# BraveenSri/siddhi

Measured on AMD Instinct MI355X. Metric: events/sec (whole node) for partitioned pattern query at 1/2/4/8 GPUs; % HBM peak, higher is better.
Workload: dtype f32

## Files before the change

### siddhi_amd/csrc/gwalk.h

```cpp
#pragma once
#include <hip/hip_runtime.h>

#include <algorithm>
#include <cstdlib>
#include <cstring>
#include <type_traits>

#include "keypart.h"
#include "sg_engine.h"
#include "sg_prim.h"
#include "walk.h"

struct GwArgs {
  int64_t n, nc;
  int64_t within;
  int64_t t0;
  uint32_t K, ns1;
  int32_t stack_mode;
  int32_t cap;
  int32_t chunk;
  int32_t carry_out;
  int32_t pzero;
  const uint32_t* o1;
  const PtU4* grec;
  const uint8_t* glk;
  const uint32_t* kbase;
  uint64_t* trig;
  uint32_t epoch;
  uint64_t* area;
  int64_t* cv_ts;
  int32_t* cv_key;
  int64_t* cv_val;
  int64_t* cv_pay;
  uint32_t* cv_n;
  uint32_t cv_cap;
  uint32_t* flags;
  uint32_t* ovf_keys;
  uint32_t* ovf_n;
  uint32_t ovf_cap;
  uint32_t* match_n;
};
static const uint32_t GW_ORDER = 1, GW_OVERFLOW = 2, GW_INTERNAL = 4, GW_CARRY_FULL = 8;

static const uint32_t GW_MATCH_MAX = (1u << 24) - 1;
__device__ __forceinline__ uint64_t gw_trig_word(uint64_t unit, uint32_t m, uint32_t epoch) {
  return unit | ((uint64_t)m << 32) | ((uint64_t)epoch << 56);
}
__device__ __forceinline__ uint32_t gw_trig_matches(uint64_t w, uint32_t epoch) {
  return (uint32_t)(w >> 56) == epoch ? (uint32_t)(w >> 32) & GW_MATCH_MAX : 0u;
}

static __global__ void __launch_bounds__(256) k_gw_count(const uint32_t* __restrict__ o1, uint32_t ns1, uint32_t K,
                                                         const uint8_t* __restrict__ glk, uint32_t* __restrict__ kcnt) {
  __shared__ uint32_t c[4][256];
  const uint32_t g = blockIdx.x, t = threadIdx.x, w = t >> 6;
#pragma unroll
  for (int q = 0; q < 4; ++q) c[q][t] = 0;
  __syncthreads();
  const uint32_t lo = o1[(size_t)g * ns1], hi = o1[(size_t)(g + 1) * ns1];
  for (uint32_t p = lo + t; p < hi; p += 256) atomicAdd(&c[w][glk[p]], 1u);
  __syncthreads();
  const uint32_t k = (g << 8) + t;
  if (k < K) kcnt[k] = c[0][t] + c[1][t] + c[2][t] + c[3][t];
}

template <int PT>
struct GwLds {
  PtU4 stage[256 * PT];
  uint32_t cw[4][256];
  uint32_t ls[256], tot[256];
  uint32_t wsum[4];
};

template <class T>
struct GwLdsRing {
  T* v;
  int32_t* t;
  int32_t* p;
  uint32_t cmask, lane;
  __device__ __forceinline__ uint32_t ix(uint32_t s) const { return (s & cmask) * 256 + lane; }
  __device__ __forceinline__ bool full(uint32_t head, uint32_t top) const { return top - head == cmask + 1; }
};
template <class T>
struct GwHbmRing {
  T* v;
  int32_t* t;
  int32_t* p;
  __device__ __forceinline__ uint32_t ix(uint32_t s) const { return s; }
  __device__ __forceinline__ bool full(uint32_t, uint32_t) const { return false; }
};

template <class T, int OP, bool STACK, class RING>
struct GwLane {
  RING R;
  uint32_t head = 0, top = 0;
  int32_t hts = 0, prev = INT32_MIN;
  T tv = T();
  bool bad = false;
  bool big = false;
  uint64_t cur = 0;
  uint32_t k = 0;
  uint32_t nm = 0;
  uint32_t wi = 0;
  __device__ __forceinline__ bool step(const GwArgs& a, const PtU4& q) {
    const int32_t dts = (int32_t)q.x;
    const uint32_t rowf = q.y;
    T x;
    const uint32_t xb = q.z;
    __builtin_memcpy(&x, &xb, sizeof(T));
    const int32_t pay = (int32_t)q.w;
    const uint32_t f = rowf >> 30;
    bad |= dts < prev;
    prev = dts;
    if (!f) return true;
    const bool live = !is_nan_val<T>(x);
    if (head != top && (uint32_t)(dts - hts) > wi) {
// ... 42 lines not shown
              R.p[wx] = R.p[si];
            }
            ++wr;
          }
        }
        top = wr;
        if (head != top) {
          hts = R.t[R.ix(head)];
          tv = R.v[R.ix(top - 1)];
        }
      }
      if (emit && m) {
        const uint64_t b = r - (uint32_t)a.nc;
        a.area[hdr] = (uint64_t)(uint32_t)dts | ((uint64_t)k << 32);
        a.area[hdr + 1] = (uint64_t)(uint32_t)val_bits<T>(x) | ((uint64_t)(uint32_t)pay << 32);
        big |= m > GW_MATCH_MAX;
        a.trig[b] = gw_trig_word(hdr, m & GW_MATCH_MAX, a.epoch);
        cur = hdr + 2 + m;
        nm += m;
      }
    }
    if ((f & F_CAND) && live) {
      if (R.full(head, top)) return false;
      const uint32_t s = R.ix(top);
      R.v[s] = x;
      R.t[s] = dts;
      R.p[s] = pay;
      if (top == head) hts = dts;
      tv = x;
      ++top;
    }
    return true;
  }
  __device__ __forceinline__ void carry(const GwArgs& a, uint32_t o) const {
    for (uint32_t e = 0; e < top - head; ++e) {
      const uint32_t s = R.ix(head + e);
      a.cv_ts[o + e] = a.t0 + (int64_t)R.t[s];
      a.cv_key[o + e] = (int32_t)k;
      a.cv_val[o + e] = val_bits<T>(R.v[s]);
      a.cv_pay[o + e] = a.pzero ? (int64_t)(uint32_t)R.p[s] : (int64_t)R.p[s];
    }
  }
};

template <class T, int OP, int PT, bool STACK>
__global__ void __launch_bounds__(256, 1) k_gwalk(GwArgs a) {
  extern __shared__ __attribute__((aligned(16))) char lds_raw[];
  GwLds<PT>& L = *(GwLds<PT>*)lds_raw;
  const uint32_t cap = (uint32_t)a.cap;
  const uint32_t t = threadIdx.x, w = t >> 6, lane = t & 63;
  const uint32_t g = xcd_block(blockIdx.x, gridDim.x);
  const uint32_t k = (g << 8) + t;
  const bool active = k < a.K;
  const uint32_t lo = a.o1[(size_t)g * a.ns1], hi = a.o1[(size_t)(g + 1) * a.ns1];
  GwLane<T, OP, STACK, GwLdsRing<T>> W;
  W.R.v = (T*)(lds_raw + sizeof(GwLds<PT>));
  W.R.t = (int32_t*)(W.R.v + (size_t)cap * 256);
  W.R.p = W.R.t + (size_t)cap * 256;
  W.R.cmask = cap - 1;
  W.R.lane = t;
  W.k = k;
  W.wi = a.within > 0xffffffffll ? 0xffffffffu : (uint32_t)a.within;
  W.cur = active ? 3ull * a.kbase[k] : 0ull;
  bool ovf = false;
  const uint32_t ROWS = 256 * PT;
  PtU4 rc[PT], rn[PT];
  uint32_t tg[PT], tn[PT];
  auto load = [&](uint32_t base, PtU4* r, uint32_t* d) {
    const uint32_t rows = min(ROWS, hi - base);
#pragma unroll
    for (int s = 0; s < PT; ++s) {
      const uint32_t i = w * (PT * 64) + s * 64 + lane;
      const uint32_t p = base + (i < rows ? i : rows - 1);
      r[s] = __builtin_nontemporal_load(a.grec + p);
      d[s] = a.glk[p];
    }
  };
  if (lo < hi) load(lo, rc, tg);
  for (uint32_t base = lo; base < hi; base += ROWS) {
    {
      const uint32_t rows = min(ROWS, hi - base);
#pragma unroll
      for (int s = 0; s < PT; ++s)
        if (w * (PT * 64) + s * 64 + lane >= rows) tg[s] = 0xffffffffu;
    }
#pragma unroll
    for (int q = 0; q < 4; ++q) L.cw[q][t] = 0;
    __syncthreads();
#pragma unroll
    for (int s = 0; s < PT; ++s)
      if (tg[s] != 0xffffffffu) atomicAdd(&L.cw[w][tg[s]], 1u);
    __syncthreads();
    {
      const uint32_t c0 = L.cw[0][t], c1 = L.cw[1][t], c2 = L.cw[2][t], c3 = L.cw[3][t];
      const uint32_t tt = c0 + c1 + c2 + c3;
      const uint32_t ex = block_excl_scan256(tt, L.wsum);
      L.ls[t] = ex;
      L.tot[t] = tt;
      L.cw[0][t] = ex;
      L.cw[1][t] = ex + c0;
      L.cw[2][t] = ex + c0 + c1;
      L.cw[3][t] = ex + c0 + c1 + c2;
    }
    __syncthreads();
#pragma unroll
    for (int s = 0; s < PT; ++s) {
      const bool valid = tg[s] != 0xffffffffu;
// ... 9 lines not shown
    if (base + ROWS < hi) load(base + ROWS, rn, tn);
    __syncthreads();
    const uint32_t i0 = L.ls[t], i1 = i0 + L.tot[t];
    for (uint32_t i = i0; i < i1 && active && !ovf; ++i)
      if (!W.step(a, L.stage[i])) ovf = true;
    __syncthreads();
#pragma unroll
    for (int s = 0; s < PT; ++s) { rc[s] = rn[s]; tg[s] = tn[s]; }
  }
  uint32_t fl = W.bad ? GW_ORDER : 0u;
  if (active && W.cur > 3ull * a.kbase[k + 1]) fl |= GW_INTERNAL;
  if (ovf) {
    const uint32_t o = atomicAdd(a.ovf_n, 1u);
    if (o < a.ovf_cap) a.ovf_keys[o] = k;
    else fl |= GW_OVERFLOW;
  }
  if (fl) atomicOr(a.flags, fl);
  {
    uint32_t c = (active && !ovf) ? W.nm : 0u;
#pragma unroll
    for (int o = 32; o > 0; o >>= 1) c += (uint32_t)__shfl_xor((int)c, o);
    if (lane == 0 && c) atomicAdd(a.match_n, c);
  }
  if (!a.carry_out) return;
  const uint32_t m = (active && !ovf) ? W.top - W.head : 0u;
  uint32_t incl = m;
#pragma unroll
  for (int o = 1; o < 64; o <<= 1) {
    const uint32_t y = (uint32_t)__shfl_up((int)incl, o);
    if ((int)lane >= o) incl += y;
  }
  const uint32_t tot = (uint32_t)__shfl((int)incl, 63);
  if (!tot) return;
  uint32_t cb = 0;
  if (lane == 63) cb = atomicAdd(a.cv_n, tot);
  cb = (uint32_t)__shfl((int)cb, 63);
  if ((uint64_t)cb + tot > (uint64_t)a.cv_cap) {
    if (lane == 63) atomicOr(a.flags, GW_CARRY_FULL);
    return;
  }
  if (m) W.carry(a, cb + incl - m);
}

static const uint32_t GW_REDO_LDS = 2048;
template <class T, int OP, bool STACK>
__global__ void __launch_bounds__(256) k_gw_redo(GwArgs a, uint32_t* __restrict__ rows, T* __restrict__ hv,
                                                 int32_t* __restrict__ ht, int32_t* __restrict__ hp) {
  __shared__ uint32_t wc[4], base_s;
  __shared__ PtU4 red_stage[GW_REDO_LDS];
  __shared__ T red_v[GW_REDO_LDS];
  __shared__ int32_t red_t[GW_REDO_LDS], red_p[GW_REDO_LDS];
  const uint32_t k = a.ovf_keys[blockIdx.x];
  const uint32_t g = k >> 8, d = k & 255u, t = threadIdx.x, w = t >> 6, lane = t & 63;
  const uint32_t lo = a.o1[(size_t)g * a.ns1], hi = a.o1[(size_t)(g + 1) * a.ns1];
  const uint32_t kb = a.kbase[k], ke = a.kbase[k + 1];
  if (t == 0) base_s = 0;
  __syncthreads();
  for (uint32_t p0 = lo; p0 < hi; p0 += 256) {
    const uint32_t p = p0 + t;
    const bool mine = p < hi && a.glk[p] == d;
    const uint64_t bm = __ballot(mine);
    const uint32_t below = __builtin_amdgcn_mbcnt_hi((uint32_t)(bm >> 32), __builtin_amdgcn_mbcnt_lo((uint32_t)bm, 0u));
    if (lane == 0) wc[w] = (uint32_t)__popcll(bm);
    __syncthreads();
    uint32_t before = base_s;
    for (uint32_t q = 0; q < w; ++q) before += wc[q];
    if (mine && kb + before + below < ke) rows[kb + before + below] = p;
    __syncthreads();
    if (t == 0) base_s += wc[0] + wc[1] + wc[2] + wc[3];
    __syncthreads();
  }
  const uint32_t nk = ke - kb;
  const bool in_lds = nk <= GW_REDO_LDS;
  if (in_lds)
    for (uint32_t i = t; i < nk; i += 256) red_stage[i] = a.grec[rows[kb + i]];
  __syncthreads();
  if (t != 0) return;
  if (kb + base_s != ke) { atomicOr(a.flags, GW_INTERNAL); return; }
  GwLane<T, OP, STACK, GwHbmRing<T>> W;
  if (in_lds) {
    W.R.v = red_v;
    W.R.t = red_t;
    W.R.p = red_p;
  } else {
    W.R.v = hv + kb;
    W.R.t = ht + kb;
    W.R.p = hp + kb;
  }
  W.k = k;
  W.wi = a.within > 0xffffffffll ? 0xffffffffu : (uint32_t)a.within;
  W.cur = 3ull * kb;
  if (in_lds) for (uint32_t i = 0; i < nk; ++i) W.step(a, red_stage[i]);
  else for (uint32_t i = kb; i < ke; ++i) W.step(a, a.grec[rows[i]]);
  uint32_t fl = W.bad ? GW_ORDER : 0u;
  if (W.cur > 3ull * ke) fl |= GW_INTERNAL;
  if (W.big) fl |= GW_OVERFLOW;
  if (fl) atomicOr(a.flags, fl);
  if (W.nm) atomicAdd(a.match_n, W.nm);
  if (!a.carry_out) return;
  const uint32_t m = W.top - W.head;
  if (!m) return;
  const uint32_t o = atomicAdd(a.cv_n, m);
  if ((uint64_t)o + m > (uint64_t)a.cv_cap) { atomicOr(a.flags, GW_CARRY_FULL); return; }
  W.carry(a, o);
}

struct GwSel {
// ... 158 lines not shown
  const size_t cap = h->ws.bufs[name].bytes;
  if (p != tw.p || cap != tw.cap) {
    tw.p = p;
    tw.cap = cap;
    tw.hw = 0;
  }
  if (wrap && tw.hw) HIPCHK(hipMemsetAsync(p, 0, sizeof(uint64_t) * tw.hw, st));
  if (words > tw.hw) {
    HIPCHK(hipMemsetAsync(p + tw.hw, 0, sizeof(uint64_t) * (words - tw.hw), st));
    tw.hw = words;
  }
  return p;
}

static void gw_project(SgHandle* h, const BatchView& bv, int64_t n, const GwArgs& ga, const GwSel& sel, uint32_t total) {
  const sg_nfa_desc& d = h->desc;
  hipStream_t st = h->stream;
  char* out = h->out.reserve(total, d.n_select, st);
  const int64_t ntile = (n + GW_TILE - 1) / GW_TILE;
  uint32_t* tcount = (uint32_t*)h->ws.get("gw_tcount", sizeof(uint32_t) * ((size_t)ntile + 1), st);
  uint32_t* tbase = (uint32_t*)h->ws.get("gw_tbase", sizeof(uint32_t) * ((size_t)ntile + 1), st);
  h->kbeg("gw_tiles");
  HIPCHK(hipMemsetAsync(tcount + ntile, 0, sizeof(uint32_t), st));
  hipLaunchKernelGGL(k_gtile_count, dim3((unsigned)((ntile + 7) / 8)), dim3(256), 0, st, n, (const uint64_t*)ga.trig, ga.epoch,
                     tcount, ntile);
  HIPCHK(hipGetLastError());
  sg_exclusive_scan(h->ws, st, "gw_tscan_tmp", tcount, tbase, (uint32_t)0, (size_t)ntile + 1, rocprim::plus<uint32_t>());
  h->kend();
  uint32_t tsum = 0;
  HIPCHK(hipMemcpyAsync(&tsum, tbase + ntile, sizeof(uint32_t), hipMemcpyDeviceToHost, st));
  h->kbeg("gw_project");
  const size_t plds = (size_t)GW_PROJ_S * sel.stride;
  if (plds > 65536)
    HIPCHK(hipFuncSetAttribute((const void*)k_gscan_project, hipFuncAttributeMaxDynamicSharedMemorySize, (int)plds));
  hipLaunchKernelGGL(k_gscan_project, dim3((unsigned)ntile), dim3(256), plds, st, n, ga.t0, bv.base_index, bv.index,
                     (const uint64_t*)ga.trig, ga.epoch, (const uint64_t*)ga.area, sel, (int64_t)h->out.n, out,
                     (const uint32_t*)tbase);
  HIPCHK(hipGetLastError());
  h->kend();
  HIPCHK(hipStreamSynchronize(st));
  if (tsum != total) throw SgError(SG_EINVAL, "internal: group walker match count mismatch");
  h->out.n += total;
}

template <class T>
static int run_group_walk(SgHandle* h, const BatchView& bv, int64_t n, int64_t nc, uint32_t kb, const PartPlan& pp,
                          const uint32_t* o1, const WRec<T, true>* grec, const uint8_t* glk, uint32_t* pk_flags,
                          const GwPlan& gp, const PushPlan& plan, const Virt& v, const SgCols& cc, int op, int stack_mode,
                          int val_col_a, EveryNextState* es) {
  const sg_nfa_desc& d = h->desc;
  hipStream_t st = h->stream;
  const int64_t nt = nc + n;
  const uint32_t ng = (kb + 255) >> 8;
  uint32_t* kcnt = (uint32_t*)h->ws.get("gw_kcnt", sizeof(uint32_t) * ((size_t)kb + 1), st);
  uint32_t* kbase = (uint32_t*)h->ws.get("gw_kbase", sizeof(uint32_t) * ((size_t)kb + 1), st);
  h->kbeg("gw_count");
  HIPCHK(hipMemsetAsync(kcnt, 0, sizeof(uint32_t) * ((size_t)kb + 1), st));
  hipLaunchKernelGGL(k_gw_count, dim3(ng), dim3(256), 0, st, o1, pp.ns1, kb, glk, kcnt);
  HIPCHK(hipGetLastError());
  sg_exclusive_scan(h->ws, st, "gw_kscan_tmp", kcnt, kbase, (uint32_t)0, (size_t)kb + 1, rocprim::plus<uint32_t>());
  h->kend();
  uint32_t pkf = 0;
  int64_t t0 = 0;
  HIPCHK(hipMemcpyAsync(&pkf, pk_flags, sizeof(uint32_t), hipMemcpyDeviceToHost, st));
  HIPCHK(hipMemcpyAsync(&t0, nc ? v.c_ts : v.ts, sizeof(int64_t), hipMemcpyDeviceToHost, st));
  HIPCHK(hipStreamSynchronize(st));
  const PackRange pr = pack_range(pkf);
  if (pr == PACK_TS_RANGE) return 2;
  if (pr == PACK_PAY_RANGE) return 0;
  h->mark(2);

  GwArgs ga;
  memset(&ga, 0, sizeof(ga));
  ga.n = n;
  ga.nc = nc;
  ga.within = d.within;
  ga.t0 = t0;
  ga.K = kb;
  ga.ns1 = pp.ns1;
  ga.stack_mode = stack_mode;
  ga.cap = gp.cap;
  ga.chunk = 4096;
  ga.carry_out = h->opt.no_carry ? 0 : 1;
  ga.pzero = v.pfloat;
  ga.o1 = o1;
  ga.grec = (const PtU4*)grec;
  ga.glk = glk;
  ga.kbase = kbase;
  const char* ee = getenv("SG_DEBUG_GW_EPOCHS");
  const uint32_t epochs = ee ? (uint32_t)std::min(std::max(atoi(ee), 1), 255) : 255u;
  const bool wrap = h->gw_epoch >= epochs;
  h->gw_epoch = wrap ? 1u : h->gw_epoch + 1;
  ga.epoch = h->gw_epoch;
  ga.trig = gw_tagged_words(h, h->gw_trig, "gw_trig", (size_t)std::max<int64_t>(n, 1), wrap, st);
  ga.area = (uint64_t*)h->ws.get("gw_area", sizeof(uint64_t) * 3 * (size_t)std::max<int64_t>(nt, 1), st);
  uint32_t* gflags = (uint32_t*)h->ws.get("gw_flags", sizeof(uint32_t) * 4, st);
  ga.flags = gflags;
  ga.cv_n = gflags + 1;
  ga.ovf_n = gflags + 2;
  ga.ovf_cap = std::min<uint32_t>(kb, 1u << 16);
  ga.ovf_keys = (uint32_t*)h->ws.get("gw_ovf_keys", sizeof(uint32_t) * ga.ovf_cap, st);
  ga.match_n = gflags + 3;
  ga.cv_cap = (uint32_t)std::max<int64_t>(1, std::min<int64_t>(nt, (int64_t)kb * gp.cap + (1 << 22)));
  ga.cv_ts = (int64_t*)h->ws.get("cv_ts", sizeof(int64_t) * (size_t)ga.cv_cap, st);
  ga.cv_val = (int64_t*)h->ws.get("cv_val", sizeof(int64_t) * (size_t)ga.cv_cap, st);
  ga.cv_pay = (int64_t*)h->ws.get("cv_pay", sizeof(int64_t) * (size_t)ga.cv_cap, st);
  ga.cv_key = (int32_t*)h->ws.get("cv_key", sizeof(int32_t) * (size_t)ga.cv_cap, st);
  HIPCHK(hipMemsetAsync(gflags, 0, sizeof(uint32_t) * 4, st));
  h->kbeg("group_walk");
  dispatch_op(op, [&](auto opc) { launch_gwalk<T, decltype(opc)::value>(ga, ng, st); });
  h->kend();
  uint32_t hf[4] = {0, 0, 0, 0}, total = 0;
  HIPCHK(hipMemcpyAsync(hf, gflags, sizeof(hf), hipMemcpyDeviceToHost, st));
  HIPCHK(hipStreamSynchronize(st));
  if (hf[0] & GW_INTERNAL) throw SgError(SG_EINVAL, "internal: group walker guard tripped");
  if (hf[0]) return 0;
  if (hf[2]) {
    h->kbeg("gw_redo");
    uint32_t* rrows = (uint32_t*)h->ws.get("gw_redo_rows", sizeof(uint32_t) * (size_t)nt, st);
    char* rl = (char*)h->ws.get("gw_redo_list", (sizeof(T) + 8) * (size_t)nt, st);
    T* hv = (T*)rl;
    int32_t* ht = (int32_t*)(rl + sizeof(T) * (size_t)nt);
    int32_t* hp = ht + nt;
    dispatch_op(op, [&](auto opc) { launch_gw_redo<T, decltype(opc)::value>(ga, hf[2], rrows, hv, ht, hp, st); });
    h->kend();
    HIPCHK(hipMemcpyAsync(hf, gflags, sizeof(hf), hipMemcpyDeviceToHost, st));
    HIPCHK(hipStreamSynchronize(st));
    if (hf[0] & GW_INTERNAL) throw SgError(SG_EINVAL, "internal: group walker redo guard tripped");
    if (hf[0]) return 0;
  }
  h->last_spilled = hf[2];
  total = hf[3];
// ... 28 lines not shown
```

### siddhi_amd/csrc/keypart.h

```cpp
#pragma once
#include <hip/hip_runtime.h>

#include <algorithm>
#include <cstdlib>
#include <cstring>
#include <type_traits>

#include "sg_engine.h"
#include "sg_prim.h"
#include "walk_rec.h"

#ifndef SG_PT1
#define SG_PT1 4
#endif
#ifndef SG_PT2
#define SG_PT2 16
#endif
static const int PT1 = SG_PT1, PT1_ROWS = 256 * SG_PT1;
static const int PT2 = SG_PT2, PT2_ROWS = 256 * SG_PT2;
static const int PT_D = 256;

struct PartPlan {
  uint32_t K, lb, ng, two;
  uint32_t nb1, nb2;
  uint32_t seg1, ns1;
  uint32_t ts2, nj;
};

template <class R, int PT, class TG = uint16_t>
struct PartLds {
  R stage[256 * PT];
  TG tag[256 * PT];
  uint32_t cw[4][PT_D];
  uint32_t ls[PT_D];
  uint32_t tot[PT_D];
  uint32_t run[PT_D];
  uint32_t wsum[4];
};

__device__ __forceinline__ uint32_t block_excl_scan256(uint32_t x, uint32_t* wsum) {
  const int lane = threadIdx.x & 63, w = threadIdx.x >> 6;
  uint32_t inc = x;
#pragma unroll
  for (int o = 1; o < 64; o <<= 1) {
    const uint32_t y = (uint32_t)__shfl_up((int)inc, o);
    if (lane >= o) inc += y;
  }
  if (lane == 63) wsum[w] = inc;
  __syncthreads();
  uint32_t add = 0;
  for (int i = 0; i < w; ++i) add += wsum[i];
  return add + inc - x;
}

__device__ __forceinline__ void peer_rank(bool valid, uint32_t d, uint32_t nb, uint32_t& rank, uint32_t& cnt) {
  uint64_t m = __ballot(valid);
  for (uint32_t b = 0; b < nb; ++b) {
    const bool bit = (d >> b) & 1u;
    const uint64_t bb = __ballot(bit);
    m &= bit ? bb : ~bb;
  }
  rank = __builtin_amdgcn_mbcnt_hi((uint32_t)(m >> 32), __builtin_amdgcn_mbcnt_lo((uint32_t)m, 0u));
  cnt = (uint32_t)__popcll(m);
}

template <class R, int PT, class TG>
__device__ __forceinline__ uint32_t part_cursors(PartLds<R, PT, TG>& L) {
  const uint32_t t = threadIdx.x;
  const uint32_t c0 = L.cw[0][t], c1 = L.cw[1][t], c2 = L.cw[2][t], c3 = L.cw[3][t];
  const uint32_t tot = c0 + c1 + c2 + c3;
  const uint32_t ex = block_excl_scan256(tot, L.wsum);
  L.ls[t] = ex;
  L.tot[t] = tot;
  L.cw[0][t] = ex;
  L.cw[1][t] = ex + c0;
  L.cw[2][t] = ex + c0 + c1;
  L.cw[3][t] = ex + c0 + c1 + c2;
  __syncthreads();
  return L.ls[PT_D - 1] + L.tot[PT_D - 1];
// ... 69 lines not shown
            if (R::has_pay && pk.v.pcol && pk.v.pw == 8) {
              const int64_t pv = v_payload(pk.v, r);
              if (pv != (int64_t)(int32_t)pv) bad |= PK_PAY_RANGE;
            }
          }
        }
      }
    }
  };
  uint32_t tg[P], tn[P];
  R rc[P], rn[P];
  if (rb < re) load(rb, tg, rc);
  for (int64_t base = rb; base < re; base += PROWS) {
#pragma unroll
    for (int q = 0; q < 4; ++q) L.cw[q][t] = 0;
    __syncthreads();
#pragma unroll
    for (int s = 0; s < P; ++s)
      if (tg[s] != 0xffffffffu) atomicAdd(&L.cw[w][tg[s] >> pp.lb], 1u);
    __syncthreads();
    const uint32_t staged = part_cursors(L);
#pragma unroll
    for (int s = 0; s < P; ++s) {
      const bool valid = tg[s] != 0xffffffffu;
      const uint32_t d = valid ? tg[s] >> pp.lb : 0u;
      uint32_t rank, cnt;
      peer_rank(valid, d, pp.nb1, rank, cnt);
      if (valid) {
        const uint32_t slot = L.cw[w][d] + rank;
        if (rank == 0) L.cw[w][d] = slot + cnt;
        L.stage[slot] = rc[s];
        L.tag[slot] = (TG)tg[s];
      }
    }
    if (base + PROWS < re) load(base + PROWS, tn, rn);
    __syncthreads();
    for (uint32_t q = t; q < staged; q += 256) {
      const uint32_t k = L.tag[q], d = k >> pp.lb;
      const uint32_t dst = L.run[d] + q - L.ls[d];
      if ((int64_t)dst >= nt) { bad |= PK_INTERNAL; continue; }
      orec[dst] = L.stage[q];
      if (olk) olk[dst] = (LK)(k & lmask);
    }
    __syncthreads();
    L.run[t] += L.tot[t];
#pragma unroll
    for (int s = 0; s < P; ++s) { tg[s] = tn[s]; rc[s] = rn[s]; }
  }
  if (bad) atomicOr(flags, bad);
}

__device__ __forceinline__ void part2_range(const PartPlan& pp, const uint32_t* o1, uint32_t g, uint32_t jj,
                                            uint32_t& lo, uint32_t& hi) {
  lo = o1[(size_t)g * pp.ns1 + jj * pp.ts2];
  hi = o1[(size_t)g * pp.ns1 + min(pp.ns1, (jj + 1) * pp.ts2)];
}

static __global__ void __launch_bounds__(256) k_part2_hist(PartPlan pp, const uint32_t* __restrict__ o1,
                                                           const uint8_t* __restrict__ glk, uint32_t* __restrict__ h2) {
  __shared__ uint32_t cnt[4][PT_D];
  const uint32_t g = blockIdx.x / pp.nj, jj = blockIdx.x % pp.nj, t = threadIdx.x, w = t >> 6;
#pragma unroll
  for (int q = 0; q < 4; ++q) cnt[q][t] = 0;
  __syncthreads();
  uint32_t lo, hi;
  part2_range(pp, o1, g, jj, lo, hi);
  for (uint32_t pb = lo; pb < hi; pb += 256 * 8) {
    uint32_t d[8];
#pragma unroll
    for (int s = 0; s < 8; ++s) {
      const uint32_t p = pb + s * 256 + t;
      d[s] = p < hi ? (uint32_t)glk[p] : 0xffffffffu;
    }
#pragma unroll
    for (int s = 0; s < 8; ++s)
      if (d[s] != 0xffffffffu) atomicAdd(&cnt[w][d[s]], 1u);
  }
  __syncthreads();
  if (t < (1u << pp.lb)) h2[(size_t)((g << pp.lb) + t) * pp.nj + jj] = cnt[0][t] + cnt[1][t] + cnt[2][t] + cnt[3][t];
}

template <class R>
__global__ void __launch_bounds__(256) k_part2(PartPlan pp, const uint32_t* __restrict__ o1, const uint32_t* __restrict__ o2,
                                               const R* __restrict__ grec, const uint8_t* __restrict__ glk,
                                               R* __restrict__ srec, uint32_t cap, uint32_t* __restrict__ flags) {
  extern __shared__ __attribute__((aligned(16))) char lds_raw[];
  PartLds<R, PT2>& L = *(PartLds<R, PT2>*)lds_raw;
  const uint32_t g = blockIdx.x / pp.nj, jj = blockIdx.x % pp.nj;
  const uint32_t t = threadIdx.x, w = t >> 6, lane = t & 63;
  if (t < (1u << pp.lb)) L.run[t] = o2[(size_t)((g << pp.lb) + t) * pp.nj + jj];
  uint32_t lo, hi;
  part2_range(pp, o1, g, jj, lo, hi);
  auto load = [&](uint32_t base, uint32_t* tg, R* rc) {
    const uint32_t rows = (hi - base < (uint32_t)PT2_ROWS) ? hi - base : (uint32_t)PT2_ROWS;
#pragma unroll
    for (int s = 0; s < PT2; ++s) {
      const uint32_t i = w * (PT2 * 64) + s * 64 + lane;
      const uint32_t p = base + (i < rows ? i : rows - 1);
      const uint32_t lk = glk[p];
      rc[s] = grec[p];
      tg[s] = i < rows ? lk : 0xffffffffu;
    }
  };
  uint32_t tg[PT2], tn[PT2];
  R rc[PT2], rn[PT2];
  if (lo < hi) load(lo, tg, rc);
  for (uint32_t base = lo; base < hi; base += PT2_ROWS) {
#pragma unroll
// ... 15 lines not shown
        if (rank == 0) L.cw[w][d] = slot + cnt;
        L.stage[slot] = rc[s];
        L.tag[slot] = (uint16_t)d;
      }
    }
    if (hi - base > (uint32_t)PT2_ROWS) load(base + PT2_ROWS, tn, rn);
    __syncthreads();
    for (uint32_t q = t; q < staged; q += 256) {
      const uint32_t d = L.tag[q];
      const uint32_t dst = L.run[d] + q - L.ls[d];
      if (dst >= cap) { atomicOr(flags, PK_INTERNAL); continue; }
      srec[dst] = L.stage[q];
    }
    __syncthreads();
    L.run[t] += L.tot[t];
#pragma unroll
    for (int s = 0; s < PT2; ++s) { tg[s] = tn[s]; rc[s] = rn[s]; }
  }
}

typedef uint32_t PtU4 __attribute__((ext_vector_type(4)));
struct PtB24 { uint64_t a, b, c; };
template <class R>
using PtRaw = typename std::conditional<sizeof(R) == 16, PtU4, PtB24>::type;

static __global__ void k_part_segs(uint32_t K, const uint32_t* __restrict__ o, uint32_t stride,
                                   uint32_t* __restrict__ seg_b, uint32_t* __restrict__ seg_e) {
  const uint32_t k = blockIdx.x * blockDim.x + threadIdx.x;
  if (k >= K) return;
  seg_b[k] = o[(size_t)k * stride];
  seg_e[k] = o[(size_t)(k + 1) * stride];
}

static PartPlan part_plan(uint32_t K, int64_t nt) {
  PartPlan p;
  memset(&p, 0, sizeof(p));
  p.K = K;
  uint32_t bits = 0;
  while ((1ull << bits) < (uint64_t)K) ++bits;
  auto nbits = [](uint32_t nd) { uint32_t b = 0; while ((1u << b) < nd) ++b; return b; };
  if (K <= (uint32_t)PT_D) {
    p.two = 0; p.lb = 0; p.ng = K;
  } else {
    const uint32_t hb = (bits + 1) / 2;
    p.two = 1; p.lb = bits - hb; p.ng = (K + (1u << p.lb) - 1) >> p.lb;
  }
  p.nb1 = nbits(p.ng);
  p.nb2 = p.lb;
  const int64_t sub = std::max<int64_t>(1, std::min<int64_t>(32, nt / ((int64_t)PT1_ROWS * 2048)));
  p.seg1 = (uint32_t)(PT1_ROWS * sub);
  p.ns1 = (uint32_t)std::max<int64_t>(1, (nt + p.seg1 - 1) / p.seg1);
  p.ts2 = (uint32_t)std::max<int64_t>(1, std::min<int64_t>(p.ns1, (int64_t)8192 * p.ng / p.seg1));
  p.nj = (p.ns1 + p.ts2 - 1) / p.ts2;
  return p;
}


static __global__ void __launch_bounds__(256) k_hist_wide(KeyOf kf, uint32_t K, uint32_t lb, uint32_t ng, uint32_t seg1,
                                                          uint32_t ns1, int64_t nt, uint32_t* __restrict__ h,
                                                          uint32_t lbs, uint32_t nsg, uint32_t* __restrict__ ha,
                                                          uint32_t* __restrict__ flags) {
  __shared__ uint32_t cnt[4096];
  const uint32_t j = blockIdx.x, t = threadIdx.x;
  for (uint32_t g = t; g < ng; g += 256) cnt[g] = 0;
  __syncthreads();
  const int64_t r0 = (int64_t)j * seg1, r1 = min(nt, r0 + seg1);
  uint32_t bad = 0;
  for (int64_t rb = r0; rb < r1; rb += 256 * 8) {
    uint32_t k[8];
#pragma unroll
    for (int s = 0; s < 8; ++s) {
      const int64_t r = rb + s * 256 + t;
      k[s] = r < r1 ? kf((uint32_t)r) : 0xffffffffu;
    }
#pragma unroll
    for (int s = 0; s < 8; ++s) {
      if (k[s] < K) atomicAdd(&cnt[k[s] >> lb], 1u);
      else if (k[s] != 0xffffffffu) bad |= PK_KEY_RANGE;
    }
  }
  __syncthreads();
  for (uint32_t g = t; g < ng; g += 256) h[(size_t)g * ns1 + j] = cnt[g];
  for (uint32_t sg = t; sg < nsg; sg += 256) {
    uint32_t c = 0;
    for (uint32_t g = sg << lbs; g < ((sg + 1) << lbs) && g < ng; ++g) c += cnt[g];
    ha[(size_t)sg * ns1 + j] = c;
  }
  if (bad) atomicOr(flags, bad);
}

struct Part1bArgs {
  uint32_t lb;
  uint32_t lbs;
  uint32_t ns1, tsb;
  uint32_t nsb;
  const uint32_t* oa;
  const uint32_t* o1;
};

template <int PT>
struct Part1bLds {
  PtU4 stage[256 * PT];
  uint16_t tag[256 * PT];
  uint32_t cw[4][256];
  uint32_t ls[256], tot[256], run[256];
  uint32_t wsum[4];
};

template <int PT>
__global__ void __launch_bounds__(256) k_part1b(Part1bArgs B, const PtU4* __restrict__ grecA, const uint16_t* __restrict__ glkA,
                                                PtU4* __restrict__ grec, uint8_t* __restrict__ glk, uint32_t cap,
                                                uint32_t* __restrict__ flags) {
  extern __shared__ __attribute__((aligned(16))) char lds_raw[];
  Part1bLds<PT>& L = *(Part1bLds<PT>*)lds_raw;
  const uint32_t sg = blockIdx.x / B.nsb, jj = blockIdx.x % B.nsb;
  const uint32_t t = threadIdx.x, w = t >> 6, lane = t & 63;
  const uint32_t jf = min(B.ns1, jj * B.tsb), jl = min(B.ns1, jf + B.tsb);
  const uint32_t lo = B.oa[(size_t)sg * B.ns1 + jf], hi = B.oa[(size_t)sg * B.ns1 + jl];
  const uint32_t nd = 1u << B.lbs, lmask = (1u << B.lb) - 1u;
  if (t < nd) L.run[t] = B.o1[(size_t)((sg << B.lbs) | t) * B.ns1 + jf];
  const int ROWS = 256 * PT;
  auto load = [&](uint32_t base, PtU4* rc, uint32_t* tg) {
    const uint32_t rows = min((uint32_t)ROWS, hi - base);
#pragma unroll
    for (int s = 0; s < PT; ++s) {
      const uint32_t i = w * (PT * 64) + s * 64 + lane;
      const uint32_t p = base + (i < rows ? i : rows - 1);
      rc[s] = grecA[p];
      const uint32_t k = glkA[p];
      tg[s] = i < rows ? k : 0xffffffffu;
    }
  };
  PtU4 rc[PT], rn[PT];
  uint32_t tg[PT], tn[PT];
  if (lo < hi) load(lo, rc, tg);
  for (uint32_t base = lo; base < hi; base += ROWS) {
#pragma unroll
    for (int q = 0; q < 4; ++q) L.cw[q][t] = 0;
    __syncthreads();
#pragma unroll
    for (int s = 0; s < PT; ++s)
      if (tg[s] != 0xffffffffu) atomicAdd(&L.cw[w][tg[s] >> B.lb], 1u);
    __syncthreads();
    uint32_t staged;
    {
      const uint32_t c0 = L.cw[0][t], c1 = L.cw[1][t], c2 = L.cw[2][t], c3 = L.cw[3][t];
      const uint32_t tt = c0 + c1 + c2 + c3;
      const uint32_t ex = block_excl_scan256(tt, L.wsum);
      L.ls[t] = ex;
      L.tot[t] = tt;
      L.cw[0][t] = ex;
      L.cw[1][t] = ex + c0;
      L.cw[2][t] = ex + c0 + c1;
      L.cw[3][t] = ex + c0 + c1 + c2;
      __syncthreads();
      staged = L.ls[255] + L.tot[255];
    }
#pragma unroll
    for (int s = 0; s < PT; ++s) {
      const bool valid = tg[s] != 0xffffffffu;
      const uint32_t d = valid ? tg[s] >> B.lb : 0u;
      uint32_t rank, cnt;
      peer_rank(valid, d, B.lbs, rank, cnt);
      if (valid) {
        const uint32_t slot = L.cw[w][d] + rank;
        if (rank == 0) L.cw[w][d] = slot + cnt;
        L.stage[slot] = rc[s];
        L.tag[slot] = (uint16_t)tg[s];
      }
    }
    if (base + ROWS < hi) load(base + ROWS, rn, tn);
    __syncthreads();
    for (uint32_t q = t; q < staged; q += 256) {
      const uint32_t k = L.tag[q], d = k >> B.lb;
      const uint32_t dst = L.run[d] + q - L.ls[d];
      if (dst >= cap) { atomicOr(flags, PK_INTERNAL); continue; }
      grec[dst] = L.stage[q];
      glk[dst] = (uint8_t)(k & lmask);
    }
    __syncthreads();
    if (t < nd) L.run[t] += L.tot[t];
#pragma unroll
    for (int s = 0; s < PT; ++s) { rc[s] = rn[s]; tg[s] = tn[s]; }
  }
}

template <class T>
static void part1_wide(SgHandle* h, const PackFn<T, true>& pk, KeyOf kf, uint32_t kb, int64_t nt, const PartPlan& pp,
                       uint32_t* h1, uint32_t* o1, WRec<T, true>* grec, uint8_t* glk, uint32_t* pk_flags) {
  typedef WRec<T, true> R;
  hipStream_t st = h->stream;
  const uint32_t lb = pp.lb, ng = pp.ng;
  const size_t n1 = (size_t)pp.ng * pp.ns1 + 1;
  {
    uint32_t lbs = 0;
    while (((ng + (1u << lbs) - 1) >> lbs) > 64u && lbs < 8) ++lbs;
    PartPlan pa2 = pp;
    pa2.lb = lb + lbs;
    pa2.ng = (kb + (1u << pa2.lb) - 1) >> pa2.lb;
    uint32_t nbA = 0;
    while ((1u << nbA) < pa2.ng) ++nbA;
    pa2.nb1 = nbA;
    const size_t nA = (size_t)pa2.ng * pp.ns1 + 1;
    uint32_t* hA = (uint32_t*)h->ws.get("part_hA", sizeof(uint32_t) * nA, st);
    uint32_t* oA = (uint32_t*)h->ws.get("part_oA", sizeof(uint32_t) * nA, st);
    R* grecA = (R*)h->ws.get("grecA", sizeof(R) * nt, st);
    uint16_t* glkA = (uint16_t*)h->ws.get("glkA", 2 * nt, st);
    h->kbeg("part_hist");
    HIPCHK(hipMemsetAsync(hA + nA - 1, 0, sizeof(uint32_t), st));
    HIPCHK(hipMemsetAsync(h1 + n1 - 1, 0, sizeof(uint32_t), st));
    hipLaunchKernelGGL(k_hist_wide, dim3(pp.ns1), dim3(256), 0, st, kf, kb, lb, ng, pp.seg1, pp.ns1, nt, h1, lbs, pa2.ng, hA,
                       pk_flags);
    HIPCHK(hipGetLastError());
    sg_exclusive_scan(h->ws, st, "part_scan_tmpA", (const uint32_t*)hA, oA, (uint32_t)0, nA, rocprim::plus<uint32_t>());
    sg_exclusive_scan(h->ws, st, "part_scan_tmp", (const uint32_t*)h1, o1, (uint32_t)0, n1, rocprim::plus<uint32_t>());
    h->kend();
    h->kbeg("part_group");
    const char* pe = getenv("SG_DEBUG_P1_PT");
    const int p1 = pe ? atoi(pe) : 8;
    auto launch_a = [&](auto pt) {
      constexpr int P = decltype(pt)::value;
      const size_t ldsA = sizeof(PartLds<R, P, uint32_t>);
      HIPCHK(hipFuncSetAttribute((const void*)k_part1<T, true, uint32_t, uint16_t, P>,
                                 hipFuncAttributeMaxDynamicSharedMemorySize, (int)ldsA));
      hipLaunchKernelGGL((k_part1<T, true, uint32_t, uint16_t, P>), dim3(pp.ns1), dim3(256), ldsA, st, pk, kf, pa2, nt, oA,
                         grecA, glkA, pk_flags);
    };
    if (p1 == 8) launch_a(std::integral_constant<int, 8>());
    else if (p1 == 16) launch_a(std::integral_constant<int, 16>());
    else launch_a(std::integral_constant<int, PT1>());
    HIPCHK(hipGetLastError());
    h->kend();
    h->kbeg("part_split");
    Part1bArgs B;
    B.lb = lb;
    B.lbs = lbs;
    B.ns1 = pp.ns1;
    const int64_t per_sg = std::max<int64_t>(1, nt / pa2.ng);
    B.nsb = (uint32_t)std::max<int64_t>(1, std::min<int64_t>(pp.ns1, per_sg / 32768));
    B.tsb = (pp.ns1 + B.nsb - 1) / B.nsb;
    B.nsb = (pp.ns1 + B.tsb - 1) / B.tsb;
    B.oa = oA;
    B.o1 = o1;
    const size_t ldsB = sizeof(Part1bLds<16>);
    HIPCHK(hipFuncSetAttribute((const void*)k_part1b<16>, hipFuncAttributeMaxDynamicSharedMemorySize, (int)ldsB));
    hipLaunchKernelGGL((k_part1b<16>), dim3(pa2.ng * B.nsb), dim3(256), ldsB, st, B, (const PtU4*)grecA, glkA,
                       (PtU4*)grec, glk, (uint32_t)nt, pk_flags);
    HIPCHK(hipGetLastError());
    h->kend();
  }
}


struct PushCtx {
  SgHandle* h;
  const BatchView& bv;
  int64_t n, nc, nt;
  uint32_t kb, K;
  int op, val_col_a, val_col_b;
  KeyOf kf;
};

template <class T, bool N>
struct KeyPart {
  Src<T, N> src;
  uint32_t* seg_b;
  uint32_t* seg_e;
  uint32_t* pk_flags;
  WRec<T, N>* prec;
};

template <class T, bool N>
static KeyPart<T, N> part_begin(const PushCtx& c, const Virt& v) {
  typedef WRec<T, N> R;
  SgHandle* h = c.h;
  hipStream_t st = h->stream;
  KeyPart<T, N> kp;
  kp.src.srec = nullptr;
  kp.src.pk.v = v;
  kp.pk_flags = (uint32_t*)h->ws.get("pack_flags", sizeof(uint32_t), st);
  HIPCHK(hipMemsetAsync(kp.pk_flags, 0, sizeof(uint32_t), st));
  kp.prec = (R*)h->ws.get("prec", sizeof(R) * c.nt, st);
  kp.seg_b = (uint32_t*)h->ws.get("seg_b", sizeof(uint32_t) * c.K, st);
  kp.seg_e = (uint32_t*)h->ws.get("seg_e", sizeof(uint32_t) * c.K, st);
  return kp;
}

template <class T, bool N>
struct PartLdsBufs {
  PartPlan pp;
  size_t n1, n2;
  uint32_t *h1, *o1, *h2, *o2;
  WRec<T, N>* srec;
  WRec<T, N>* grec;
  uint8_t* glk;
};
template <class T, bool N>
static PartLdsBufs<T, N> part_lds_bufs(const PushCtx& c) {
  typedef WRec<T, N> R;
  typedef PtRaw<R> RW;
  static_assert(sizeof(RW) == sizeof(R), "raw record layout");
  SgHandle* h = c.h;
  hipStream_t st = h->stream;
  PartLdsBufs<T, N> b;
  memset(&b, 0, sizeof(b));
  PartPlan& pp = b.pp;
  pp = part_plan(c.kb, c.nt);
  if (c.kb > 65536u) {
    pp.two = 1;
    pp.lb = 8;
    pp.ng = (c.kb + 255u) >> 8;
    pp.nb1 = 0;
    while ((1u << pp.nb1) < pp.ng) ++pp.nb1;
    pp.nb2 = 8;
    pp.ts2 = (uint32_t)std::max<int64_t>(1, std::min<int64_t>(pp.ns1, (int64_t)8192 * pp.ng / pp.seg1));
    pp.nj = (pp.ns1 + pp.ts2 - 1) / pp.ts2;
  }
  b.n1 = (size_t)pp.ng * pp.ns1 + 1;
  b.h1 = (uint32_t*)h->ws.get("part_h1", sizeof(uint32_t) * b.n1, st);
  b.o1 = (uint32_t*)h->ws.get("part_o1", sizeof(uint32_t) * b.n1, st);
  b.srec = (R*)h->ws.get("srec", sizeof(R) * c.nt, st);
  HIPCHK(hipFuncSetAttribute((const void*)k_part1<T, N>, hipFuncAttributeMaxDynamicSharedMemorySize,
                             (int)sizeof(PartLds<R, PT1>)));
  HIPCHK(hipFuncSetAttribute((const void*)k_part2<RW>, hipFuncAttributeMaxDynamicSharedMemorySize,
                             (int)sizeof(PartLds<RW, PT2>)));
  if (pp.two) {
    b.grec = (R*)h->ws.get("grec", sizeof(R) * c.nt, st);
    b.glk = (uint8_t*)h->ws.get("glk", c.nt, st);
    b.n2 = ((size_t)pp.ng << pp.lb) * pp.nj + 1;
    b.h2 = (uint32_t*)h->ws.get("part_h2", sizeof(uint32_t) * b.n2, st);
    b.o2 = (uint32_t*)h->ws.get("part_o2", sizeof(uint32_t) * b.n2, st);
  }
  return b;
}

template <class T, bool N>
static void part_lds_pass1(const PushCtx& c, KeyPart<T, N>& kp, const PartLdsBufs<T, N>& b) {
  SgHandle* h = c.h;
  hipStream_t st = h->stream;
  const PartPlan& pp = b.pp;
  const size_t lds1 = sizeof(PartLds<WRec<T, N>, PT1>);
  h->kbeg("part_hist");
  HIPCHK(hipMemsetAsync(b.h1 + b.n1 - 1, 0, sizeof(uint32_t), st));
  hipLaunchKernelGGL(k_part1_hist, dim3(pp.ns1), dim3(256), 0, st, c.kf, pp, c.nt, b.h1, kp.pk_flags);
  HIPCHK(hipGetLastError());
  sg_exclusive_scan(h->ws, st, "part_scan_tmp", b.h1, b.o1, (uint32_t)0, b.n1, rocprim::plus<uint32_t>());
  h->kend();
  h->kbeg(pp.two ? "part_group" : "part_scatter");
  hipLaunchKernelGGL((k_part1<T, N>), dim3(pp.ns1), dim3(256), lds1, st, kp.src.pk, c.kf, pp, c.nt, b.o1,
                     pp.two ? b.grec : b.srec, b.glk, kp.pk_flags);
  HIPCHK(hipGetLastError());
  h->kend();
  if (!pp.two)
    hipLaunchKernelGGL(k_part_segs, dim3((c.kb + 255) / 256), dim3(256), 0, st, c.kb, b.o1, pp.ns1, kp.seg_b, kp.seg_e);
}

template <class T, bool N>
static void part_lds_pass2(const PushCtx& c, KeyPart<T, N>& kp, const PartLdsBufs<T, N>& b) {
  typedef PtRaw<WRec<T, N>> RW;
  SgHandle* h = c.h;
  hipStream_t st = h->stream;
  const PartPlan& pp = b.pp;
  h->kbeg("part_hist2");
  HIPCHK(hipMemsetAsync(b.h2 + b.n2 - 1, 0, sizeof(uint32_t), st));
  hipLaunchKernelGGL(k_part2_hist, dim3(pp.ng * pp.nj), dim3(256), 0, st, pp, b.o1, b.glk, b.h2);
  HIPCHK(hipGetLastError());
  sg_exclusive_scan(h->ws, st, "part_scan_tmp2", b.h2, b.o2, (uint32_t)0, b.n2, rocprim::plus<uint32_t>());
  h->kend();
  h->kbeg("part_key");
  hipLaunchKernelGGL((k_part2<RW>), dim3(pp.ng * pp.nj), dim3(256), sizeof(PartLds<RW, PT2>), st, pp, b.o1, b.o2,
                     (const RW*)b.grec, b.glk, (RW*)b.srec, (uint32_t)c.nt, kp.pk_flags);
// ... 50 lines not shown
```

Before: 16.05 billion.

## Coarsen partition histogram columns and fuse key-base scan into count kernel

```diff
diff --git a/siddhi_amd/csrc/gwalk.h b/siddhi_amd/csrc/gwalk.h
--- a/siddhi_amd/csrc/gwalk.h
+++ b/siddhi_amd/csrc/gwalk.h
@@ -15,7 +15,7 @@
   int64_t n, nc;
   int64_t within;
   int64_t t0;
-  uint32_t K, ns1;
+  uint32_t K, nc1;
   int32_t stack_mode;
   int32_t cap;
   int32_t chunk;
@@ -50,18 +50,41 @@
   return (uint32_t)(w >> 56) == epoch ? (uint32_t)(w >> 32) & GW_MATCH_MAX : 0u;
 }
 
-static __global__ void __launch_bounds__(256) k_gw_count(const uint32_t* __restrict__ o1, uint32_t ns1, uint32_t K,
-                                                         const uint8_t* __restrict__ glk, uint32_t* __restrict__ kcnt) {
+static __global__ void __launch_bounds__(256) k_gw_count(const uint32_t* __restrict__ o1, uint32_t nc1, uint32_t K,
+                                                         const uint8_t* __restrict__ glk, uint32_t* __restrict__ kbase) {
   __shared__ uint32_t c[4][256];
+  __shared__ uint32_t wsum[4];
   const uint32_t g = blockIdx.x, t = threadIdx.x, w = t >> 6;
 #pragma unroll
   for (int q = 0; q < 4; ++q) c[q][t] = 0;
   __syncthreads();
-  const uint32_t lo = o1[(size_t)g * ns1], hi = o1[(size_t)(g + 1) * ns1];
-  for (uint32_t p = lo + t; p < hi; p += 256) atomicAdd(&c[w][glk[p]], 1u);
+  const uint32_t lo = o1[(size_t)g * nc1], hi = o1[(size_t)(g + 1) * nc1];
+  const uint32_t mis = (uint32_t)(16u - ((uintptr_t)(glk + lo) & 15u)) & 15u;
+  const uint32_t a0 = min(hi, lo + mis);
+  const uint32_t nv = (hi - a0) >> 4;
+  const uint32_t a1 = a0 + (nv << 4);
+  if (t < a0 - lo) atomicAdd(&c[w][glk[lo + t]], 1u);
+  if (t < hi - a1) atomicAdd(&c[w][glk[a1 + t]], 1u);
+  const PtU4* v = (const PtU4*)(glk + a0);
+  auto count = [&](const PtU4& x) {
+#pragma unroll
+    for (int q = 0; q < 4; ++q)
+#pragma unroll
+      for (int b = 0; b < 32; b += 8) atomicAdd(&c[w][(x[q] >> b) & 255u], 1u);
+  };
+  for (uint32_t i = t; i < nv; i += 512) {
+    const PtU4 x0 = v[i];
+    const bool two = i + 256 < nv;
+    const PtU4 x1 = v[two ? i + 256 : i];
+    count(x0);
+    if (two) count(x1);
+  }
   __syncthreads();
+  const uint32_t n = c[0][t] + c[1][t] + c[2][t] + c[3][t];
+  const uint32_t first = lo + block_excl_scan256(n, wsum);
   const uint32_t k = (g << 8) + t;
-  if (k < K) kcnt[k] = c[0][t] + c[1][t] + c[2][t] + c[3][t];
+  if (k < K) kbase[k] = first;
+  if (k + 1 == K) kbase[K] = first + n;
 }
 
 template <int PT>
@@ -210,7 +233,7 @@
   const uint32_t g = xcd_block(blockIdx.x, gridDim.x);
   const uint32_t k = (g << 8) + t;
   const bool active = k < a.K;
-  const uint32_t lo = a.o1[(size_t)g * a.ns1], hi = a.o1[(size_t)(g + 1) * a.ns1];
+  const uint32_t lo = a.o1[(size_t)g * a.nc1], hi = a.o1[(size_t)(g + 1) * a.nc1];
   GwLane<T, OP, STACK, GwLdsRing<T>> W;
   W.R.v = (T*)(lds_raw + sizeof(GwLds<PT>));
   W.R.t = (int32_t*)(W.R.v + (size_t)cap * 256);
@@ -326,7 +349,7 @@
   __shared__ int32_t red_t[GW_REDO_LDS], red_p[GW_REDO_LDS];
   const uint32_t k = a.ovf_keys[blockIdx.x];
   const uint32_t g = k >> 8, d = k & 255u, t = threadIdx.x, w = t >> 6, lane = t & 63;
-  const uint32_t lo = a.o1[(size_t)g * a.ns1], hi = a.o1[(size_t)(g + 1) * a.ns1];
+  const uint32_t lo = a.o1[(size_t)g * a.nc1], hi = a.o1[(size_t)(g + 1) * a.nc1];
   const uint32_t kb = a.kbase[k], ke = a.kbase[k + 1];
   if (t == 0) base_s = 0;
   __syncthreads();
@@ -591,13 +614,10 @@
   hipStream_t st = h->stream;
   const int64_t nt = nc + n;
   const uint32_t ng = (kb + 255) >> 8;
-  uint32_t* kcnt = (uint32_t*)h->ws.get("gw_kcnt", sizeof(uint32_t) * ((size_t)kb + 1), st);
   uint32_t* kbase = (uint32_t*)h->ws.get("gw_kbase", sizeof(uint32_t) * ((size_t)kb + 1), st);
   h->kbeg("gw_count");
-  HIPCHK(hipMemsetAsync(kcnt, 0, sizeof(uint32_t) * ((size_t)kb + 1), st));
-  hipLaunchKernelGGL(k_gw_count, dim3(ng), dim3(256), 0, st, o1, pp.ns1, kb, glk, kcnt);
+  hipLaunchKernelGGL(k_gw_count, dim3(ng), dim3(256), 0, st, o1, pp.nc1, kb, glk, kbase);
   HIPCHK(hipGetLastError());
-  sg_exclusive_scan(h->ws, st, "gw_kscan_tmp", kcnt, kbase, (uint32_t)0, (size_t)kb + 1, rocprim::plus<uint32_t>());
   h->kend();
   uint32_t pkf = 0;
   int64_t t0 = 0;
@@ -616,7 +636,7 @@
   ga.within = d.within;
   ga.t0 = t0;
   ga.K = kb;
-  ga.ns1 = pp.ns1;
+  ga.nc1 = pp.nc1;
   ga.stack_mode = stack_mode;
   ga.cap = gp.cap;
   ga.chunk = 4096;
diff --git a/siddhi_amd/csrc/keypart.h b/siddhi_amd/csrc/keypart.h
--- a/siddhi_amd/csrc/keypart.h
+++ b/siddhi_amd/csrc/keypart.h
@@ -25,6 +25,7 @@
   uint32_t nb1, nb2;
   uint32_t seg1, ns1;
   uint32_t ts2, nj;
+  uint32_t w1, nc1;
 };
 
 template <class R, int PT, class TG = uint16_t>
@@ -200,8 +201,9 @@
 
 __device__ __forceinline__ void part2_range(const PartPlan& pp, const uint32_t* o1, uint32_t g, uint32_t jj,
                                             uint32_t& lo, uint32_t& hi) {
-  lo = o1[(size_t)g * pp.ns1 + jj * pp.ts2];
-  hi = o1[(size_t)g * pp.ns1 + min(pp.ns1, (jj + 1) * pp.ts2)];
+  const uint32_t cs = pp.ts2 / pp.w1;
+  lo = o1[(size_t)g * pp.nc1 + jj * cs];
+  hi = o1[(size_t)g * pp.nc1 + min(pp.nc1, (jj + 1) * cs)];
 }
 
 static __global__ void __launch_bounds__(256) k_part2_hist(PartPlan pp, const uint32_t* __restrict__ o1,
@@ -323,40 +325,57 @@
   p.ns1 = (uint32_t)std::max<int64_t>(1, (nt + p.seg1 - 1) / p.seg1);
   p.ts2 = (uint32_t)std::max<int64_t>(1, std::min<int64_t>(p.ns1, (int64_t)8192 * p.ng / p.seg1));
   p.nj = (p.ns1 + p.ts2 - 1) / p.ts2;
+  p.w1 = 1;
+  p.nc1 = p.ns1;
   return p;
 }
 
+static const uint32_t P1_COL_SEGS = 8;
 
 static __global__ void __launch_bounds__(256) k_hist_wide(KeyOf kf, uint32_t K, uint32_t lb, uint32_t ng, uint32_t seg1,
-                                                          uint32_t ns1, int64_t nt, uint32_t* __restrict__ h,
-                                                          uint32_t lbs, uint32_t nsg, uint32_t* __restrict__ ha,
-                                                          uint32_t* __restrict__ flags) {
+                                                          uint32_t ns1, uint32_t w1, uint32_t nc1, int64_t nt,
+                                                          uint32_t* __restrict__ h, uint32_t lbs, uint32_t nsg,
+                                                          uint32_t* __restrict__ ha, uint32_t* __restrict__ flags) {
   __shared__ uint32_t cnt[4096];
-  const uint32_t j = blockIdx.x, t = threadIdx.x;
+  __shared__ uint32_t sgc[64];
+  const uint32_t jj = blockIdx.x, t = threadIdx.x, w = t >> 6, lane = t & 63;
   for (uint32_t g = t; g < ng; g += 256) cnt[g] = 0;
+  if (t < 64) sgc[t] = 0;
   __syncthreads();
-  const int64_t r0 = (int64_t)j * seg1, r1 = min(nt, r0 + seg1);
   uint32_t bad = 0;
-  for (int64_t rb = r0; rb < r1; rb += 256 * 8) {
-    uint32_t k[8];
-#pragma unroll
-    for (int s = 0; s < 8; ++s) {
-      const int64_t r = rb + s * 256 + t;
-      k[s] = r < r1 ? kf((uint32_t)r) : 0xffffffffu;
-    }
-#pragma unroll
-    for (int s = 0; s < 8; ++s) {
-      if (k[s] < K) atomicAdd(&cnt[k[s] >> lb], 1u);
-      else if (k[s] != 0xffffffffu) bad |= PK_KEY_RANGE;
-    }
-  }
-  __syncthreads();
-  for (uint32_t g = t; g < ng; g += 256) h[(size_t)g * ns1 + j] = cnt[g];
-  for (uint32_t sg = t; sg < nsg; sg += 256) {
-    uint32_t c = 0;
-    for (uint32_t g = sg << lbs; g < ((sg + 1) << lbs) && g < ng; ++g) c += cnt[g];
-    ha[(size_t)sg * ns1 + j] = c;
-  }
+  const uint32_t j1 = min(ns1, (jj + 1) * w1), nd = 1u << lbs;
+  for (uint32_t j = jj * w1; j < j1; ++j) {
+    const int64_t r0 = (int64_t)j * seg1, r1 = min(nt, r0 + seg1);
+    for (int64_t rb = r0; rb < r1; rb += 256 * 8) {
+      uint32_t k[8];
+#pragma unroll
+      for (int s = 0; s < 8; ++s) {
+        const int64_t r = rb + s * 256 + t;
+        k[s] = r < r1 ? kf((uint32_t)r) : 0xffffffffu;
+      }
+#pragma unroll
+      for (int s = 0; s < 8; ++s) {
+        if (k[s] < K) atomicAdd(&cnt[k[s] >> lb], 1u);
+        else if (k[s] != 0xffffffffu) bad |= PK_KEY_RANGE;
+      }
+    }
+    __syncthreads();
+    for (uint32_t sg = w; sg < nsg; sg += 4) {
+      uint32_t c = 0;
+      for (uint32_t i = lane; i < nd; i += 64) {
+        const uint32_t g = (sg << lbs) + i;
+        c += g < ng ? cnt[g] : 0u;
+      }
+#pragma unroll
+      for (int o = 32; o > 0; o >>= 1) c += (uint32_t)__shfl_xor((int)c, o);
+      if (lane == 0) {
+        ha[(size_t)sg * ns1 + j] = c - sgc[sg];
+        sgc[sg] = c;
+      }
+    }
+    __syncthreads();
+  }
+  for (uint32_t g = t; g < ng; g += 256) h[(size_t)g * nc1 + jj] = cnt[g];
   if (bad) atomicOr(flags, bad);
 }
 
@@ -365,6 +384,7 @@
   uint32_t lbs;
   uint32_t ns1, tsb;
   uint32_t nsb;
+  uint32_t ng, w1, nc1;
   const uint32_t* oa;
   const uint32_t* o1;
 };
@@ -389,7 +409,7 @@
   const uint32_t jf = min(B.ns1, jj * B.tsb), jl = min(B.ns1, jf + B.tsb);
   const uint32_t lo = B.oa[(size_t)sg * B.ns1 + jf], hi = B.oa[(size_t)sg * B.ns1 + jl];
   const uint32_t nd = 1u << B.lbs, lmask = (1u << B.lb) - 1u;
-  if (t < nd) L.run[t] = B.o1[(size_t)((sg << B.lbs) | t) * B.ns1 + jf];
+  if (t < nd && ((sg << B.lbs) | t) < B.ng) L.run[t] = B.o1[(size_t)((sg << B.lbs) | t) * B.nc1 + jf / B.w1];
   const int ROWS = 256 * PT;
   auto load = [&](uint32_t base, PtU4* rc, uint32_t* tg) {
     const uint32_t rows = min((uint32_t)ROWS, hi - base);
@@ -462,7 +482,7 @@
   typedef WRec<T, true> R;
   hipStream_t st = h->stream;
   const uint32_t lb = pp.lb, ng = pp.ng;
-  const size_t n1 = (size_t)pp.ng * pp.ns1 + 1;
+  const size_t n1 = (size_t)pp.ng * pp.nc1 + 1;
   {
     uint32_t lbs = 0;
     while (((ng + (1u << lbs) - 1) >> lbs) > 64u && lbs < 8) ++lbs;
@@ -480,8 +500,8 @@
     h->kbeg("part_hist");
     HIPCHK(hipMemsetAsync(hA + nA - 1, 0, sizeof(uint32_t), st));
     HIPCHK(hipMemsetAsync(h1 + n1 - 1, 0, sizeof(uint32_t), st));
-    hipLaunchKernelGGL(k_hist_wide, dim3(pp.ns1), dim3(256), 0, st, kf, kb, lb, ng, pp.seg1, pp.ns1, nt, h1, lbs, pa2.ng, hA,
-                       pk_flags);
+    hipLaunchKernelGGL(k_hist_wide, dim3(pp.nc1), dim3(256), 0, st, kf, kb, lb, ng, pp.seg1, pp.ns1, pp.w1, pp.nc1, nt, h1,
+                       lbs, pa2.ng, hA, pk_flags);
     HIPCHK(hipGetLastError());
     sg_exclusive_scan(h->ws, st, "part_scan_tmpA", (const uint32_t*)hA, oA, (uint32_t)0, nA, rocprim::plus<uint32_t>());
     sg_exclusive_scan(h->ws, st, "part_scan_tmp", (const uint32_t*)h1, o1, (uint32_t)0, n1, rocprim::plus<uint32_t>());
@@ -508,9 +528,15 @@
     B.lbs = lbs;
     B.ns1 = pp.ns1;
     const int64_t per_sg = std::max<int64_t>(1, nt / pa2.ng);
-    B.nsb = (uint32_t)std::max<int64_t>(1, std::min<int64_t>(pp.ns1, per_sg / 32768));
+    const char* be = getenv("SG_DEBUG_P1B_ROWS");
+    const int64_t rows_b = be ? std::max(atoi(be), 1) : 32768;
+    B.nsb = (uint32_t)std::max<int64_t>(1, std::min<int64_t>(pp.ns1, per_sg / rows_b));
     B.tsb = (pp.ns1 + B.nsb - 1) / B.nsb;
+    B.tsb = (B.tsb + pp.w1 - 1) / pp.w1 * pp.w1;
     B.nsb = (pp.ns1 + B.tsb - 1) / B.tsb;
+    B.ng = ng;
+    B.w1 = pp.w1;
+    B.nc1 = pp.nc1;
     B.oa = oA;
     B.o1 = o1;
     const size_t ldsB = sizeof(Part1bLds<16>);
@@ -584,10 +610,13 @@
     pp.nb1 = 0;
     while ((1u << pp.nb1) < pp.ng) ++pp.nb1;
     pp.nb2 = 8;
+    pp.w1 = P1_COL_SEGS;
+    pp.nc1 = (pp.ns1 + pp.w1 - 1) / pp.w1;
     pp.ts2 = (uint32_t)std::max<int64_t>(1, std::min<int64_t>(pp.ns1, (int64_t)8192 * pp.ng / pp.seg1));
+    pp.ts2 = (pp.ts2 + pp.w1 - 1) / pp.w1 * pp.w1;
     pp.nj = (pp.ns1 + pp.ts2 - 1) / pp.ts2;
   }
-  b.n1 = (size_t)pp.ng * pp.ns1 + 1;
+  b.n1 = (size_t)pp.ng * pp.nc1 + 1;
   b.h1 = (uint32_t*)h->ws.get("part_h1", sizeof(uint32_t) * b.n1, st);
   b.o1 = (uint32_t*)h->ws.get("part_o1", sizeof(uint32_t) * b.n1, st);
   b.srec = (R*)h->ws.get("srec", sizeof(R) * c.nt, st);
```

Result: faster. 16.68 billion (median of 6 runs) (+3.9%).
